# uzh-rpg/dagr

Measured on AMD Instinct MI355X. Metric: events_per_sec, higher is better.
Workload: dtype f32; 1 GPU; dagr-s + --use_image --img_net resnet50, 640x480 synthetic S-uniform, B=8 windows/step x 100000 events (50 ms each), r=7, K=16, events->graph->GNN(+image fusion)->decoded head outputs->confidence mask + NMS (device); image_branch=in-line, engines=3

## Files before the change

### dagr_amd/_lib.py

```python
import ctypes
import os

_HERE = os.path.dirname(os.path.abspath(__file__))
LIB_PATH = os.path.join(_HERE, "lib", "libdagr_hip.so")

c_void_p = ctypes.c_void_p
c_i32 = ctypes.c_int32
c_i64 = ctypes.c_int64
c_size_t = ctypes.c_size_t
c_float = ctypes.c_float


class PoolDesc(ctypes.Structure):
    _fields_ = [("batch_size", c_i32), ("channels", c_i32), ("gx", c_i32), ("gy", c_i32), ("vx", c_float),
                ("vy", c_float), ("inv_w", c_float), ("inv_h", c_float), ("two_max", c_float), ("r00", c_float),
                ("r02", c_float), ("r11", c_float), ("r12", c_float), ("rx", c_i32), ("ry", c_i32), ("aggr", c_i32),
                ("append_pos", c_i32), ("keep_order", c_i32)]


class GraphDesc(ctypes.Structure):
    _fields_ = [("width", c_i32), ("height", c_i32), ("batch_size", c_i32), ("max_neighbors", c_i32),
                ("queue_size", c_i32), ("radius", c_i32), ("delta_t_us", c_i32), ("time_window", c_i32),
                ("max_events", c_i64)]

# ... 111 lines not shown
    "dagr_pool_argmax": (ctypes.c_int, [c_void_p, c_i32, c_void_p, c_i32, c_i32, c_void_p, c_i32, c_i32, c_void_p, c_void_p]),
    "dagr_pool_grad": (ctypes.c_int, [c_void_p, c_i32, c_i32, c_i32, c_void_p, c_void_p, c_void_p, c_i32, c_void_p, c_i32,
                                      c_void_p]),
    "dagr_to_dense_grad": (ctypes.c_int, [c_i32, c_i32, c_void_p, c_void_p, c_float, c_float, c_i32, c_i32, c_i32, c_void_p,
                                          c_void_p, c_i32, c_void_p]),
    "dagr_sample_features": (ctypes.c_int, [c_void_p, c_i32, c_void_p, c_void_p, c_i32, c_void_p, c_i32, c_i32, c_i32,
                                            c_i32, c_i32, c_i32, c_void_p, c_i32, c_i32, c_void_p]),
    "dagr_nms_batched": (ctypes.c_int, [c_void_p, c_void_p, c_void_p, c_void_p, c_i32, c_i32, c_float, c_float, c_void_p,
                                        c_void_p, c_void_p, c_void_p]),
    "dagr_heads_finish": (ctypes.c_int, [ctypes.POINTER(HeadScale), ctypes.POINTER(HeadScale), c_i32, c_i32, c_void_p,
                                         c_void_p, c_void_p]),
    "dagr_heads_finish_detect": (ctypes.c_int, [ctypes.POINTER(HeadScale), ctypes.POINTER(HeadScale), c_i32, c_i32, c_void_p,
                                                c_void_p, c_float, c_float, c_float, c_void_p, c_void_p, c_void_p]),
    "dagr_decode_heads": (ctypes.c_int, [c_void_p, c_i32, c_i32, c_float, c_void_p, c_i32, c_i32, c_float, c_i32, c_i32,
                                         c_void_p, c_void_p]),
    "dagr_postprocess": (ctypes.c_int, [c_void_p, c_i32, c_i32, c_i32, c_float, c_float, c_float, c_void_p, c_void_p,
                                        c_void_p]),
    "dagr_masked_lin": (ctypes.c_int, [c_void_p, c_void_p, c_void_p, c_void_p, c_void_p, c_i32, c_i64, c_i32, c_i32, c_void_p]),
    "dagr_masked_lin_no_bias": (ctypes.c_int, [c_void_p, c_void_p, c_void_p, c_void_p, c_i32, c_i64, c_i32, c_i32, c_void_p]),
    "dagr_masked_isdiff": (ctypes.c_int, [c_void_p, c_void_p, c_void_p, c_float, c_float, c_i64, c_i32, c_void_p]),
    "dagr_masked_inplace_BN": (ctypes.c_int, [c_void_p, c_void_p, c_void_p, c_void_p, c_void_p, c_void_p, c_void_p, c_float,
                                              c_i64, c_i32, c_void_p]),
    "dagr_downsample_events": (ctypes.c_int, [c_void_p, c_void_p, c_void_p, c_i32, c_void_p, c_i32, c_i32, c_void_p,
                                              c_void_p, c_void_p]),
    "dagr_spline_conv_l0_tiles_rows": (ctypes.c_int, [c_i32, c_i32, c_i32, c_i32, c_i32, c_i32, c_i32, c_i32, c_i32, c_float,
                                                      c_float, c_i64, c_i64, c_i32, c_void_p, c_void_p, c_void_p, c_void_p,
                                                      c_i32, c_void_p, c_i32, c_void_p, c_void_p, c_i32, c_void_p, c_i32,
                                                      c_void_p, c_void_p]),
    "dagr_async_graph_append": (ctypes.c_int, [ctypes.POINTER(GraphDesc), c_void_p, c_i64, c_i64, c_void_p, c_void_p,
                                               c_void_p, c_i64, c_void_p, c_i32, c_void_p, c_i32, c_i64, c_void_p, c_void_p,
                                               c_void_p, c_void_p, c_void_p, c_void_p, c_void_p, c_void_p, c_void_p, c_i32,
                                               c_i32, c_i32, c_void_p]),
    "dagr_async_update": (ctypes.c_int, [ctypes.POINTER(AsyncUpdateArgs), c_void_p]),
    "dagr_pool_l0_stream": (ctypes.c_int, [ctypes.POINTER(PoolDesc), c_void_p, c_i32, ctypes.POINTER(GraphDesc), c_void_p,
                                           c_void_p, c_void_p, c_void_p, c_i32, c_void_p, c_void_p, c_i64, c_i64, c_i64,
                                           c_void_p, c_void_p, c_void_p, c_void_p, c_i32, c_i32, c_void_p, c_void_p,
                                           c_void_p, c_void_p, c_void_p, c_void_p, c_void_p, c_i32, c_void_p]),
    "dagr_spline_conv_fused_lds_bytes": (c_size_t, [c_i32, c_i32]),
    "dagr_spline_conv_fused_passes": (c_i32, [c_i32, c_i32]),
    "dagr_spline_conv_fused": (ctypes.c_int, [c_void_p, c_i32, c_void_p, c_void_p, c_void_p, c_void_p, c_i32, c_i32,
                                              c_void_p, c_i32, c_i32, c_i32, c_i32, c_float, c_float, c_void_p,
                                              c_void_p, c_void_p, c_i32, c_i32, c_i32, c_void_p]),
    "dagr_spline_conv_fused_pool": (ctypes.c_int, [c_void_p, c_i32, c_void_p, c_void_p, c_void_p, c_void_p, c_i32, c_i32,
                                                   c_void_p, c_i32, c_i32, c_i32, c_i32, c_float, c_float, c_void_p,
                                                   c_void_p, c_void_p, c_i32, c_i32, c_i32, ctypes.POINTER(PoolDesc),
                                                   c_void_p, c_void_p, c_void_p, c_void_p, c_void_p]),
    "dagr_spline_conv_fused_multi": (ctypes.c_int, [c_void_p, c_i32, c_void_p]),
    "dagr_spline_conv_fused_pair": (ctypes.c_int, [c_void_p, c_i32, c_void_p, c_void_p, c_void_p, c_i32, c_i32, c_i32, c_i32,
                                                   c_float, c_float, c_i32, c_i32, c_void_p, c_void_p, c_void_p, c_void_p,
                                                   c_i32, c_void_p, c_void_p, c_void_p, c_void_p, c_i32, c_void_p]),
    "dagr_gemm_epilogue_workspace_bytes": (c_size_t, []),
    "dagr_gemm_epilogue": (ctypes.c_int, [c_void_p, c_i64, c_i32, c_i64, c_void_p, c_i32, c_void_p, c_void_p, c_i64, c_i32,
                                          c_void_p, c_i64, c_void_p, c_size_t, c_void_p]),
    "dagr_add_relu": (ctypes.c_int, [c_void_p, c_void_p, c_i64, c_void_p]),
    "dagr_bias_relu": (ctypes.c_int, [c_void_p, c_void_p, c_i64, c_i32, c_void_p]),
    "dagr_bias_silu": (ctypes.c_int, [c_void_p, c_void_p, c_i64, c_i32, c_void_p]),
    "dagr_bn_relu_maxpool": (ctypes.c_int, [c_void_p, c_i32, c_i32, c_i32, c_i32, c_void_p, c_void_p, c_void_p, c_void_p]),
    "dagr_gemm_bias_act": (ctypes.c_int, [c_void_p, c_i32, c_void_p, c_i32, c_void_p, c_i32, c_void_p, c_void_p,
                                          c_i32, c_i32, c_i32, c_i32, c_void_p]),
    "dagr_async_flops": (ctypes.c_int, [c_void_p, c_i32, c_void_p, c_void_p, c_void_p, c_void_p, c_void_p, c_i32, c_void_p,
                                        c_void_p]),
    "dagr_viz_workspace_bytes": (c_size_t, [c_i32, c_i32, c_i32]),
    "dagr_viz_render": (ctypes.c_int, [c_void_p, c_i32, c_i32, c_i32, c_void_p, c_i32, c_void_p, c_void_p, c_void_p,
                                       c_void_p, c_i32, c_void_p, c_void_p, c_void_p, c_i32, c_i32, c_void_p, c_i32,
                                       c_void_p, c_void_p, c_void_p, c_size_t, c_void_p]),
}

_lib = None


def lib():
    global _lib
    if _lib is None:
        if not os.path.exists(LIB_PATH):
            raise RuntimeError(
                f"dagr_amd: {LIB_PATH} not found -- build it with `make` (or __graft_entry__.build()). "
                "There is no CPU fallback for the event-graph hot path.")
        handle = ctypes.CDLL(LIB_PATH)
        for name, (res, args) in SIGNATURES.items():
            fn = getattr(handle, name)
            fn.restype = res
            fn.argtypes = args
        _lib = handle
    return _lib


def check(rc, what=""):
    if rc != 0:
        msg = lib().dagr_last_error().decode("utf-8", "replace")
        raise RuntimeError(f"libdagr_hip {what} failed (status {rc}): {msg}")


def ptr(t):
    return None if t is None else c_void_p(t.data_ptr())


def cur_stream(device=None):
    import torch
    return c_void_p(torch.cuda.current_stream(device).cuda_stream)
```

### dagr_amd/csrc/common.hpp

```cpp
#pragma once
#include <hip/hip_runtime.h>
#include <stdint.h>
#include <stdio.h>
#include <stdlib.h>
#include <string>

#include "dagr_hip.h"

namespace dagr {

void set_error(const std::string &msg);

#define DAGR_CHECK_ARG(cond, msg)                                             \
    do {                                                                      \
        if (!(cond)) {                                                        \
            ::dagr::set_error(std::string(__func__) + ": " + (msg));          \
            return DAGR_ERR_INVALID_ARG;                                      \
        }                                                                     \
    } while (0)

#define DAGR_CHECK_HIP(expr)                                                  \
    do {                                                                      \
        hipError_t _e = (expr);                                               \
        if (_e != hipSuccess) {                                               \
// ... 66 lines not shown
        int n = __shfl_up(v, d, 64);
        if (lane >= d) v += n;
    }
    return v;
}

__device__ __forceinline__ int block_exclusive_scan(int v, int *smem, int &total) {
    const int lane = threadIdx.x & 63;
    const int wid = threadIdx.x >> 6;
    int incl = wave_inclusive_scan(v);
    if (lane == 63) smem[wid] = incl;
    __syncthreads();
    int w0 = smem[0], w1 = smem[1], w2 = smem[2], w3 = smem[3];
    __syncthreads();
    int base = (wid > 0 ? w0 : 0) + (wid > 1 ? w1 : 0) + (wid > 2 ? w2 : 0);
    total = w0 + w1 + w2 + w3;
    return base + incl - v;
}

struct XcdSplit {
    int first, end, stride;
};
__device__ __forceinline__ XcdSplit xcd_split(int n_items, int items_per_block, int item_in_block) {
    const int G = gridDim.x;
    const int nx = (G % 8 == 0) ? 8 : 1;
    const int xcd = blockIdx.x % nx, lb = blockIdx.x / nx, bpx = G / nx;
    const int chunk = (n_items + nx - 1) / nx;
    const int begin = xcd * chunk;
    XcdSplit s;
    s.end = min(n_items, begin + chunk);
    s.first = begin + lb * items_per_block + item_in_block;
    s.stride = bpx * items_per_block;
    return s;
}
__device__ __forceinline__ int xcd_block(int n_blocks) {
    const int bpx = (n_blocks + 7) >> 3;
    const int lb = (int)(blockIdx.x >> 3) + (int)(blockIdx.x & 7) * bpx;
    return ((int)(blockIdx.x >> 3) < bpx && lb < n_blocks) ? lb : -1;
}
inline unsigned xcd_grid(int64_t n_blocks) { return (unsigned)((n_blocks + 7) / 8 * 8); }
inline unsigned round_grid8(int64_t g) { return (unsigned)(g <= 8 ? (g < 1 ? 1 : g) : (g + 7) / 8 * 8); }

constexpr int kScanTile = 2048;
size_t scan_scratch_elems(int64_t n);
hipError_t exclusive_scan_i32(int32_t *in, int32_t *out, int64_t n, int32_t *scratch, bool zero_input,
                              hipStream_t stream);
size_t scan_chained_state_bytes(int64_t n);
hipError_t exclusive_scan_i32_chained(int32_t *in, int32_t *out, int64_t n, void *state, bool zero_input,
                                      hipStream_t stream);


hipError_t launch_gemm_mfma(const int32_t *m_ptr, int m_max, const float *A, int lda, const float *Wm, int ldw,
                            const float *bias, float *C, int ldc, int K, int N, int relu, hipStream_t stream);
const int32_t *graph_ws_node_count(const dagr_graph_desc *desc, void *workspace);
struct PixelIndex {
    const int32_t *start;
    const int2 *slot_it;
    const int32_t *slot_xyb;
    const int32_t *n_nodes;
    const int32_t *unsorted;
    int W, H;
    __host__ __device__ int segment(int x, int yb) const { return x + W * yb; }
    __host__ __device__ int row_begin(int yb) const { return W * yb; }
};
void graph_ws_index(const dagr_graph_desc *desc, void *workspace, PixelIndex *out);

}
```

### dagr_amd/csrc/gemm_lt.hip

```cpp
#include <hipblaslt/hipblaslt.h>

#include <map>
#include <tuple>

#include "common.hpp"

namespace dagr {
namespace {

struct LtPlan {
    hipblasLtMatmulDesc_t desc = nullptr;
    hipblasLtMatrixLayout_t a = nullptr, b = nullptr, c = nullptr, d = nullptr;
    hipblasLtMatmulAlgo_t algo;
    size_t workspace = 0;
};

hipblasLtHandle_t lt_handle() {
    static hipblasLtHandle_t h = [] {
        hipblasLtHandle_t hh = nullptr;
        if (hipblasLtCreate(&hh) != HIPBLAS_STATUS_SUCCESS) hh = nullptr;
        return hh;
    }();
    return h;
}

}
}

using namespace dagr;

extern "C" size_t dagr_gemm_epilogue_workspace_bytes(void) { return (size_t)64 << 20; }

extern "C" int dagr_gemm_epilogue(const float *A, int64_t M, int32_t K, int64_t lda, const float *Wt, int32_t N,
                                  const float *bias, const float *R, int64_t ldr, int32_t act, float *D, int64_t ldd,
                                  void *workspace, size_t workspace_bytes, void *stream) {
    DAGR_CHECK_ARG(M >= 0 && K >= 1 && N >= 1 && lda >= K && ldd >= N && (!R || ldr >= N) && (act == 0 || act == 1), "bad sizes");
    if (M == 0) return DAGR_OK;
    DAGR_CHECK_ARG(A && Wt && D, "NULL pointer");
    hipblasLtHandle_t h = lt_handle();
    if (!h) { set_error("dagr_gemm_epilogue: hipblasLtCreate failed"); return DAGR_ERR_HIP; }
    using Key = std::tuple<int64_t, int, int, int64_t, int64_t, int64_t, int, int, int>;
    static thread_local std::map<Key, LtPlan> plans;
    const Key key{M, K, N, lda, R ? ldr : -1, ldd, act, bias ? 1 : 0, R ? 1 : 0};
    auto it = plans.find(key);
    if (it == plans.end()) {
        LtPlan p;
#define LT_OK(expr)                                                                                        \
    do {                                                                                                   \
        if ((expr) != HIPBLAS_STATUS_SUCCESS) { set_error("dagr_gemm_epilogue: " #expr " failed"); return DAGR_ERR_HIP; } \
    } while (0)
        LT_OK(hipblasLtMatmulDescCreate(&p.desc, HIPBLAS_COMPUTE_32F, HIP_R_32F));
        const hipblasOperation_t op_n = HIPBLAS_OP_N;
        LT_OK(hipblasLtMatmulDescSetAttribute(p.desc, HIPBLASLT_MATMUL_DESC_TRANSA, &op_n, sizeof(op_n)));
        LT_OK(hipblasLtMatmulDescSetAttribute(p.desc, HIPBLASLT_MATMUL_DESC_TRANSB, &op_n, sizeof(op_n)));
        hipblasLtEpilogue_t epi = act ? (bias ? HIPBLASLT_EPILOGUE_RELU_BIAS : HIPBLASLT_EPILOGUE_RELU)
                                      : (bias ? HIPBLASLT_EPILOGUE_BIAS : HIPBLASLT_EPILOGUE_DEFAULT);
        LT_OK(hipblasLtMatmulDescSetAttribute(p.desc, HIPBLASLT_MATMUL_DESC_EPILOGUE, &epi, sizeof(epi)));
        if (bias) {
            const hipDataType bt = HIP_R_32F;
            LT_OK(hipblasLtMatmulDescSetAttribute(p.desc, HIPBLASLT_MATMUL_DESC_BIAS_DATA_TYPE, &bt, sizeof(bt)));
            LT_OK(hipblasLtMatmulDescSetAttribute(p.desc, HIPBLASLT_MATMUL_DESC_BIAS_POINTER, &bias, sizeof(bias)));
        }
        LT_OK(hipblasLtMatrixLayoutCreate(&p.a, HIP_R_32F, (uint64_t)N, (uint64_t)K, (int64_t)N));
        LT_OK(hipblasLtMatrixLayoutCreate(&p.b, HIP_R_32F, (uint64_t)K, (uint64_t)M, lda));
        LT_OK(hipblasLtMatrixLayoutCreate(&p.c, HIP_R_32F, (uint64_t)N, (uint64_t)M, R ? ldr : ldd));
        LT_OK(hipblasLtMatrixLayoutCreate(&p.d, HIP_R_32F, (uint64_t)N, (uint64_t)M, ldd));
        hipblasLtMatmulPreference_t pref = nullptr;
        LT_OK(hipblasLtMatmulPreferenceCreate(&pref));
        const uint64_t max_ws = workspace ? (uint64_t)workspace_bytes : 0;
        LT_OK(hipblasLtMatmulPreferenceSetAttribute(pref, HIPBLASLT_MATMUL_PREF_MAX_WORKSPACE_BYTES, &max_ws, sizeof(max_ws)));
        constexpr int kCand = 16;
        hipblasLtMatmulHeuristicResult_t res[kCand];
        int found = 0;
        const hipblasStatus_t st = hipblasLtMatmulAlgoGetHeuristic(h, p.desc, p.a, p.b, p.c, p.d, pref, kCand, res, &found);
        hipblasLtMatmulPreferenceDestroy(pref);
        if (st != HIPBLAS_STATUS_SUCCESS || found < 1) {
            set_error("dagr_gemm_epilogue: the library offers no kernel for this GEMM + epilogue");
            return DAGR_ERR_UNSUPPORTED;
        }
        int best = 0;
        hipStreamCaptureStatus cap = hipStreamCaptureStatusNone;
        (void)hipStreamIsCapturing((hipStream_t)stream, &cap);
        if (found > 1 && cap == hipStreamCaptureStatusNone) {
            hipEvent_t e0, e1;
            if (hipEventCreate(&e0) == hipSuccess && hipEventCreate(&e1) == hipSuccess) {
                const float alpha = 1.0f, beta = R ? 1.0f : 0.0f;
                float best_ms = 0.f;
                for (int c = 0; c < found; c++) {
                    if (res[c].workspaceSize > workspace_bytes) continue;
                    bool ok = true;
                    float ms = 0.f;
                    for (int rep = 0; rep < 3 && ok; rep++) {
                        if (rep == 1) (void)hipEventRecord(e0, (hipStream_t)stream);
                        ok = hipblasLtMatmul(h, p.desc, &alpha, Wt, p.a, A, p.b, &beta, R ? (const void *)R : (const void *)D,
                                             p.c, D, p.d, &res[c].algo, workspace, workspace_bytes,
                                             (hipStream_t)stream) == HIPBLAS_STATUS_SUCCESS;
                    }
                    (void)hipEventRecord(e1, (hipStream_t)stream);
                    if (hipEventSynchronize(e1) != hipSuccess || !ok) continue;
                    (void)hipEventElapsedTime(&ms, e0, e1);
                    if (best_ms == 0.f || ms < best_ms) { best_ms = ms; best = c; }
                }
                (void)hipEventDestroy(e0);
                (void)hipEventDestroy(e1);
            }
        }
        p.algo = res[best].algo;
        p.workspace = res[best].workspaceSize;
        it = plans.emplace(key, p).first;
#undef LT_OK
    }
    LtPlan &p = it->second;
    if (bias && hipblasLtMatmulDescSetAttribute(p.desc, HIPBLASLT_MATMUL_DESC_BIAS_POINTER, &bias, sizeof(bias)) !=
                    HIPBLAS_STATUS_SUCCESS) {
        set_error("dagr_gemm_epilogue: setting the bias pointer failed");
        return DAGR_ERR_HIP;
    }
    DAGR_CHECK_ARG(p.workspace <= workspace_bytes, "workspace too small for the selected kernel");
    const float alpha = 1.0f, beta = R ? 1.0f : 0.0f;
    const hipblasStatus_t st = hipblasLtMatmul(h, p.desc, &alpha, Wt, p.a, A, p.b, &beta, R ? (const void *)R : (const void *)D,
                                               p.c, D, p.d, &p.algo, workspace, workspace_bytes, (hipStream_t)stream);
    if (st != HIPBLAS_STATUS_SUCCESS) {
        set_error("dagr_gemm_epilogue: hipblasLtMatmul failed");
        return DAGR_ERR_HIP;
    }
    return DAGR_OK;
}
```

### dagr_amd/engine.py

```python
import contextlib
import ctypes
import gc
import types

import numpy as np
import torch

from . import _lib
from .graph.ev_graph import WindowGraphBuilder

FUSED_PASSES_MAX_NODES = 1600


def _f32(v):
    return float(torch.as_tensor(v, dtype=torch.float32))


def _same_domain(a, b):
    return (a["rx"], a["ry"], a["den_x"], a["den_y"]) == (b["rx"], b["ry"], b["den_x"], b["den_y"]) \
        and torch.equal(a["remap"], b["remap"])


def _bn_affine(bn):
    m = bn.module
# ... 31 lines not shown
def _pack_generic(convs, norms, skip=None, relu=True, device="cuda"):
    cols, biases = [], []
    cin = convs[0].in_channels
    for conv, norm in zip(convs, norms):
        W = conv.weight.detach().float()
        root = conv.lin.weight.detach().float()
        cout = W.shape[2]
        if norm is not None:
            scale, shift = _bn_affine(norm)
        else:
            scale, shift = torch.ones(cout, device=W.device), torch.zeros(cout, device=W.device)
        if conv.bias is not None:
            shift = shift + conv.bias.detach().float() * scale
        block = torch.cat([W.reshape(25 * cin, cout), root.t()], 0) * scale.view(1, -1)
        if skip is not None:
            lin, norm_skip = skip
            s_scale, s_shift = _bn_affine(norm_skip)
            block = torch.cat([block, lin.mlp.weight.detach().float().t() * s_scale.view(1, -1)], 0)
            shift = shift + s_shift
        cols.append(block)
        biases.append(shift)
    cskip = skip[0].mlp.in_features if skip is not None else 0
    return _ConvPack(cin, cskip, torch.cat(cols, 1).to(device), torch.cat(biases).to(device), relu)


def _pack_l0(conv, norm, win, skip=None, device="cuda", cols_in=None, cols_skip=None):
    win_x, tx, win_y, ty = win
    W = conv.weight.detach().float()
    cin, cout = W.shape[1], W.shape[2]
    if cout != 16:
        raise NotImplementedError("the level-0 kernels are specialised for 16 output channels (base_width = 0.5)")
    cols_in = list(range(cin)) if cols_in is None else list(cols_in)
    scale, shift = _bn_affine(norm)
    rows = []
    for b in range(ty):
        for a in range(tx):
            rows.append(W[(win_x + a) + 5 * (win_y + b)][cols_in] * scale.view(1, -1))
    rows.append(conv.lin.weight.detach().float().t()[cols_in] * scale.view(1, -1))
    cskip = 0
    if skip is not None:
        lin, norm_skip = skip
        s_scale, s_shift = _bn_affine(norm_skip)
        ws = lin.mlp.weight.detach().float().t()
        if cols_skip is not None:
            ws = ws[list(cols_skip)]
        rows.append(ws * s_scale.view(1, -1))
        shift = shift + s_shift
        cskip = lin.mlp.in_features
    return cin, cskip, torch.cat(rows, 0).contiguous().to(device), shift.contiguous().to(device)


class _Conv1x1Gemm(torch.nn.Module):

    def __init__(self, conv, relu=False):
        super().__init__()
        cout, cin = conv.weight.shape[:2]
        self.stride = conv.stride[0]
        self.relu = relu
        self.register_buffer("wt", conv.weight.detach().reshape(cout, cin).t().contiguous())
        self.register_buffer("b", conv.bias.detach().clone() if conv.bias is not None else torch.zeros(cout, device=conv.weight.device))

    def forward(self, x, residual=None):
        if self.stride != 1:
            x = x[:, :, ::self.stride, ::self.stride]
        B, C, H, W = x.shape
        a = x.permute(0, 2, 3, 1).reshape(-1, C)
        N = self.wt.shape[1]
        r = None if residual is None else residual.permute(0, 2, 3, 1)
        if _LT["ok"] and a.is_cuda and a.dtype == torch.float32 and a.stride(1) == 1 \
                and (r is None or (r.is_contiguous() and tuple(r.shape) == (B, H, W, N))):
            y = torch.empty((a.shape[0], N), dtype=torch.float32, device=a.device)
            ws = _lt_workspace(a.device)
            act = 1 if (self.relu or r is not None) else 0
            rc = _lib.lib().dagr_gemm_epilogue(_lib.ptr(a), a.shape[0], C, a.stride(0), _lib.ptr(self.wt), N,
                                               _lib.ptr(self.b), _lib.ptr(r), N, act, _lib.ptr(y), N, _lib.ptr(ws),
                                               ws.numel(), _lib.cur_stream(a.device))
            if rc == 0:
                return y.view(B, H, W, -1).permute(0, 3, 1, 2)
            _LT["ok"] = False
        if residual is not None:
            y = torch.addmm(self.b, a, self.wt).view(B, H, W, -1).permute(0, 3, 1, 2)
            return _add_relu_(y, residual)
        y = torch._addmm_activation(self.b, a, self.wt) if self.relu else torch.addmm(self.b, a, self.wt)
        return y.view(B, H, W, -1).permute(0, 3, 1, 2)


_LT = {"ok": True, "ws": {}}


def _lt_workspace(device):
    key = str(device)
    if key not in _LT["ws"]:
        _LT["ws"][key] = torch.empty(int(_lib.lib().dagr_gemm_epilogue_workspace_bytes()), dtype=torch.uint8, device=device)
    return _LT["ws"][key]


def _gemmify_1x1(module):
    for name, child in list(module.named_children()):
        if isinstance(child, torch.nn.Conv2d) and child.kernel_size == (1, 1) and child.groups == 1 \
                and child.padding == (0, 0) and child.stride[0] == child.stride[1]:
            setattr(module, name, _Conv1x1Gemm(child))
        else:
            _gemmify_1x1(child)


def _add_relu_(y, z):
    if y.is_cuda and y.dtype == torch.float32 and z.dtype == torch.float32 and y.shape == z.shape \
            and y.stride() == z.stride() and y.data_ptr() % 16 == 0 and z.data_ptr() % 16 == 0 \
            and (y.is_contiguous() or y.is_contiguous(memory_format=torch.channels_last)):
        _lib.check(_lib.lib().dagr_add_relu(_lib.ptr(y), _lib.ptr(z), y.numel(), _lib.cur_stream(y.device)), "add_relu")
        return y
    return torch.relu_(y.add_(z))


def _bias_relu_(y, bias):
    C = y.shape[1]
    if y.is_cuda and y.dtype == torch.float32 and C % 4 == 0 and y.is_contiguous(memory_format=torch.channels_last) \
            and y.data_ptr() % 16 == 0 and bias.data_ptr() % 16 == 0:
        _lib.check(_lib.lib().dagr_bias_relu(_lib.ptr(y), _lib.ptr(bias), y.numel(), C, _lib.cur_stream(y.device)),
                   "bias_relu")
        return y
    return torch.relu_(y.add_(bias.view(1, -1, 1, 1)))


def _baseconv_forward(m, x):
    y = m.conv(x)
    b = m._bias
    C = y.shape[1]
    if y.is_cuda and y.dtype == torch.float32 and C % 4 == 0 and y.is_contiguous(memory_format=torch.channels_last) \
            and y.data_ptr() % 16 == 0 and b.data_ptr() % 16 == 0:
        _lib.check(_lib.lib().dagr_bias_silu(_lib.ptr(y), _lib.ptr(b), y.numel(), C, _lib.cur_stream(y.device)),
                   "bias_silu")
        return y
    return torch.nn.functional.silu(y.add_(b.view(1, -1, 1, 1)), inplace=True)


def _conv_bias_relu(blk, name, x):
    conv = getattr(blk, name)
    b = getattr(blk, "_" + name + "_bias", None)
    out = conv(x)
    if b is not None:
        return _bias_relu_(out, b)
    if getattr(conv, "relu", False):
        return out
    return blk.relu(out)


def _bottleneck_forward(blk, x):
    identity = x if blk.downsample is None else blk.downsample(x)
    out = _conv_bias_relu(blk, "conv1", x)
    out = _conv_bias_relu(blk, "conv2", out)
    if isinstance(blk.conv3, _Conv1x1Gemm):
        return blk.conv3(out, residual=identity)
    return _add_relu_(blk.conv3(out), identity)


def _resnet_features_forward(net, x, emit=None):
    emit = emit or (lambda name, t: None)
    c1 = net.conv1(x)
    emit("conv1", c1)
    mp = net.maxpool
    ok = (c1.is_cuda and c1.dtype == torch.float32 and c1.is_contiguous(memory_format=torch.channels_last)
          and c1.shape[1] % 4 == 0 and mp.kernel_size == 3 and mp.stride == 2 and mp.padding == 1
          and mp.dilation == 1 and not mp.ceil_mode)
    if ok:
        B, C, H, W = c1.shape
        scale, shift = net._stem_affine
        y = torch.empty((B, C, (H - 1) // 2 + 1, (W - 1) // 2 + 1), dtype=c1.dtype, device=c1.device,
                        memory_format=torch.channels_last)
        _lib.check(_lib.lib().dagr_bn_relu_maxpool(_lib.ptr(c1), B, H, W, C, _lib.ptr(scale), _lib.ptr(shift), _lib.ptr(y),
                                                   _lib.cur_stream(c1.device)), "bn_relu_maxpool")
    else:
        y = net.maxpool(net.relu(net.bn1(c1)))
    l1 = net.layer1(y)
    emit("layer1", l1)
    l2 = net.layer2(l1)
    emit("layer2", l2)
    l3 = net.layer3(l2)
    emit("layer3", l3)
    l4 = net.layer4(l3)
    emit("layer4", l4)
    return dict(conv1=c1, layer1=l1, layer2=l2, layer3=l3, layer4=l4)


def _basicblock_forward(blk, x):
    identity = x if blk.downsample is None else blk.downsample(x)
    out = _conv_bias_relu(blk, "conv1", x)
    return _add_relu_(blk.conv2(out), identity)


class _Level:

    def __init__(self, T, cin, cout, device, cf_next=0):
        self.T = T
        self.e_cap = T * 64
        i32 = dict(dtype=torch.int32, device=device)
        f32 = dict(dtype=torch.float32, device=device)
        self.x = torch.zeros((T, (cin + 3) // 4 * 4), **f32)
# ... 422 lines not shown
        if self._feat_ready is not None:
            ready = self._feat_ready.get(id(fmap))
            if ready is None:
                raise RuntimeError("pipelined window: a sampled feature map has no ready-event (the image branch did not "
                                   "announce it) -- reading it would race with the image stream")
            torch.cuda.current_stream(self.device).wait_event(ready)
        Bf, C, h, w = fmap.shape
        nhwc = fmap.permute(0, 2, 3, 1)
        if not nhwc.is_contiguous():
            nhwc = nhwc.contiguous()
        self._keep.append(nhwc)
        _lib.check(self.L.dagr_sample_features(n_ptr, n_max, _lib.ptr(pos), _lib.ptr(batch), b64, _lib.ptr(nhwc), Bf, h,
                                               w, C, self.W, self.H, _lib.ptr(out), out.shape[1], coff,
                                               _lib.cur_stream(self.device)), "sample_features")

    def _fold_image_branch(self):
        import copy
        from torch.nn.utils.fusion import fuse_conv_bn_eval
        bb, head = self.model.backbone, self.model.head
        net = copy.deepcopy(bb.net).eval()
        cnn = copy.deepcopy(head.cnn_head).eval()

        def fold_block(blk):
            for ci, bi in (("conv1", "bn1"), ("conv2", "bn2"), ("conv3", "bn3")):
                if hasattr(blk, ci):
                    setattr(blk, ci, fuse_conv_bn_eval(getattr(blk, ci), getattr(blk, bi)))
                    setattr(blk, bi, torch.nn.Identity())
            if blk.downsample is not None:
                blk.downsample = torch.nn.Sequential(fuse_conv_bn_eval(blk.downsample[0], blk.downsample[1]))
        for name in ("layer1", "layer2", "layer3", "layer4"):
            for blk in getattr(net.module, name):
                fold_block(blk)
        for m in cnn.modules():
            if hasattr(m, "conv") and hasattr(m, "bn") and isinstance(m.bn, torch.nn.BatchNorm2d):
                m.conv = fuse_conv_bn_eval(m.conv, m.bn)
                m.bn = torch.nn.Identity()
                if isinstance(getattr(m, "act", None), torch.nn.SiLU) and m.conv.bias is not None:
                    m._bias = m.conv.bias.detach().clone().contiguous()
                    m.conv.bias = None
                    m.forward = types.MethodType(_baseconv_forward, m)
        net = net.to(memory_format=torch.channels_last)
        cnn = cnn.to(memory_format=torch.channels_last)
        for blkname in ("layer1", "layer2", "layer3", "layer4"):
            _gemmify_1x1(getattr(net.module, blkname))
            for blk in getattr(net.module, blkname):
                relu_convs = ("conv1", "conv2") if hasattr(blk, "conv3") else ("conv1",)
                for cname in relu_convs:
                    conv = getattr(blk, cname)
                    if isinstance(conv, _Conv1x1Gemm):
                        conv.relu = True
                    elif isinstance(conv, torch.nn.Conv2d) and conv.bias is not None:
                        setattr(blk, "_" + cname + "_bias", conv.bias.detach().clone().contiguous())
                        conv.bias = None
                blk.forward = types.MethodType(_bottleneck_forward if hasattr(blk, "conv3") else _basicblock_forward,
                                               blk)
        bn = net.module.bn1
        scale = (bn.weight.detach().float() / torch.sqrt(bn.running_var.detach().float() + bn.eps)).contiguous()
        shift = (bn.bias.detach().float() - bn.running_mean.detach().float() * scale).contiguous()
        net.module._stem_affine = (scale, shift)
        net.module.forward_features = types.MethodType(_resnet_features_forward, net.module)
        _gemmify_1x1(net.feature_dconv)
        _gemmify_1x1(net.output_dconv)
        self._net_f, self._cnn_f = net, cnn

    def _image_branch(self, image, on_feature=None):
        if self._net_f is None:
            self._fold_image_branch()
        bb, head = types.SimpleNamespace(net=self._net_f), types.SimpleNamespace(cnn_head=self._cnn_f)
        x = image.contiguous(memory_format=torch.channels_last)
        net = self._net_f
        if on_feature is not None:
            feats = [None] * len(net.feature_layers)

            def emit(name, t):
                if name in net.feature_layers:
                    j = net.feature_layers.index(name)
                    feats[j] = net.feature_dconv[j](t) if len(net.feature_dconv) > 0 else t
                    on_feature(j, feats[j])
            d = _resnet_features_forward(net.module, x, emit)
            outs = [d[l] for l in net.output_layers]
            if len(net.output_dconv) > 0:
                outs = [dconv(o) for o, dconv in zip(outs, net.output_dconv)]
        else:
            feats, outs = bb.net(x)
        outs = outs[-self.num_scales:]
        resized = [torch.nn.functional.interpolate(f, o) for f, o in zip(outs, self.out_sizes)]
        return feats, head.cnn_head(resized)

    def stage_image(self, image):
        self._keep = []
        self._img_feats, self._cnn_out = self._image_branch(image)

    def image_async(self, image, stream=None):
        cur = torch.cuda.current_stream(self.device)
        if stream is not None:
            self._img_stream = stream
        if self._img_stream is None:
            self._img_stream = torch.cuda.Stream(self.device)
        s = self._img_stream
        s.wait_stream(cur)
        with torch.cuda.stream(s):
            feats, cnn_out = self._image_branch(image)
            ev = torch.cuda.Event()
            ev.record(s)
        return feats, cnn_out, ev

    def _consume_image_handle(self, handle):
        feats, cnn_out, ev = handle
        cur = torch.cuda.current_stream(self.device)
        cur.wait_event(ev)
        for t in list(feats) + [o for v in cnn_out.values() for o in v]:
            t.record_stream(cur)
        self._keep = []
        self._img_feats, self._cnn_out = feats, cnn_out

# ... 536 lines not shown
```

### include/dagr_hip.h

```cpp
#ifndef DAGR_HIP_H
#define DAGR_HIP_H

#include <stddef.h>
#include <stdint.h>

#ifdef __cplusplus
extern "C" {
#endif

typedef enum {
    DAGR_OK = 0,
    DAGR_ERR_INVALID_ARG = -1,
    DAGR_ERR_HIP = -2,
    DAGR_ERR_WORKSPACE = -3,
    DAGR_ERR_UNSUPPORTED = -4
} dagr_status;

const char *dagr_last_error(void);
int dagr_version(void);
int dagr_device_count(void);

int dagr_format_events(const int16_t *xy , const int32_t *t , const int8_t *p ,
                       int64_t N, int32_t width, int32_t height, int32_t time_window,
                       float *pos_out , float *feat_out , void *stream);
// ... 221 lines not shown

int dagr_add_relu(float *y, const float *z, int64_t n, void *stream);
int dagr_bias_relu(float *y_nhwc, const float *bias, int64_t n, int32_t C, void *stream);
int dagr_bias_silu(float *y_nhwc, const float *bias, int64_t n, int32_t C, void *stream);
int dagr_bn_relu_maxpool(const float *x_nhwc, int32_t B, int32_t H, int32_t W, int32_t C, const float *scale,
                         const float *shift, float *y_nhwc, void *stream);

int dagr_sample_features(const int32_t *n_ptr, int32_t n_max, const float *pos, const void *batch,
                         int32_t batch_is_int64, const float *feat_nhwc, int32_t B, int32_t h, int32_t w, int32_t C,
                         int32_t width, int32_t height, float *out, int32_t ldo, int32_t coff, void *stream);

int dagr_nms_batched(const float *boxes, const float *scores, const int32_t *cls, const uint8_t *valid,
                     int32_t B, int32_t A, float iou_threshold, float class_offset,
                     int32_t *order_out, int32_t *keep_out, int32_t *n_keep, void *stream);

typedef struct dagr_head_scale {
    const int32_t *n_ptr; int32_t n_max;
    const float *pred; int32_t ld;
    const float *pos; const int32_t *batch;
    float vx, vy, stride; int32_t Hc, Wc;
    const float *cnn[3]; int32_t cnn_stride[3][4];
    float *dense;
} dagr_head_scale;
int dagr_heads_finish(const dagr_head_scale *scale0, const dagr_head_scale *scale1, int32_t batch_size, int32_t channels,
                      float *out, int32_t *status, void *stream);
int dagr_heads_finish_detect(const dagr_head_scale *scale0, const dagr_head_scale *scale1, int32_t batch_size,
                             int32_t channels, float *out, int32_t *status, float conf_threshold, float iou_threshold,
                             float class_offset, float *det, int32_t *n_keep, void *stream);
int dagr_decode_heads(const float *dense0, int32_t H0, int32_t W0, float stride0, const float *dense1, int32_t H1,
                      int32_t W1, float stride1, int32_t B, int32_t channels, float *out, void *stream);

int dagr_postprocess(const float *pred, int32_t B, int32_t A, int32_t num_classes, float conf_threshold,
                     float iou_threshold, float class_offset, float *det, int32_t *n_keep, void *stream);

int dagr_masked_lin(const int64_t *indices, const float *x_in, float *x_out, const float *weight, const float *bias,
                    int32_t add, int64_t K, int32_t Cin, int32_t Cout, void *stream);
int dagr_masked_lin_no_bias(const int64_t *indices, const float *x_in, float *x_out, const float *weight, int32_t add,
                            int64_t K, int32_t Cin, int32_t Cout, void *stream);
int dagr_masked_isdiff(int64_t *indices, const float *x_old, const float *x_new, float atol, float rtol, int64_t K,
                       int32_t C, void *stream);
int dagr_masked_inplace_BN(const int64_t *indices, const float *x, float *x_out, const float *running_mean,
                           const float *running_var, const float *weight, const float *bias, float eps, int64_t K,
                           int32_t C, void *stream);

int dagr_downsample_events(const int32_t *order, const int32_t *run_cell, const int32_t *run_end, int32_t n_runs,
                           const int8_t *polarity, int32_t fx, int32_t fy, float *change_map, uint8_t *keep,
                           void *stream);

size_t dagr_gemm_epilogue_workspace_bytes(void);
int dagr_gemm_epilogue(const float *A, int64_t M, int32_t K, int64_t lda, const float *Wt, int32_t N, const float *bias,
                       const float *R, int64_t ldr, int32_t act, float *D, int64_t ldd, void *workspace,
                       size_t workspace_bytes, void *stream);

enum { DAGR_FLOPS_ZERO = 0, DAGR_FLOPS_CONV = 1, DAGR_FLOPS_LINEAR = 2, DAGR_FLOPS_POOL = 3, DAGR_FLOPS_CARTESIAN = 4 };
typedef struct dagr_flops_module {
    int32_t kind, level, cin, cout, root, bias;
} dagr_flops_module;
int dagr_async_flops(const int32_t *deg, int32_t n_events, const int32_t *counts1, const int32_t *counts2,
                     const int32_t *counts3, const int32_t *counts4, const dagr_flops_module *mods, int32_t n_mods,
                     int64_t *out, void *stream);

size_t dagr_viz_workspace_bytes(int32_t F, int32_t H, int32_t W);
int dagr_viz_render(const uint8_t *images, int32_t n_images, int32_t H, int32_t W, const int32_t *frame_image, int32_t F,
                    const int32_t *ev_x, const int32_t *ev_y, const int8_t *ev_p, const int32_t *ev_ptr, int32_t n_events,
                    const double *alpha, const int32_t *boxes, const int32_t *box_ptr, int32_t n_boxes, int32_t linewidth,
                    const uint8_t *colors, int32_t n_colors, uint8_t *out, int32_t *status, void *workspace,
                    size_t workspace_bytes, void *stream);

int dagr_spiral_offsets(int32_t n, int32_t *dx_host, int32_t *dy_host);

#ifdef __cplusplus
}
#endif
#endif
```

Before: 148.2 million events/s.

## Add custom MFMA implicit-GEMM conv kernel with autotuned variants for ResNet image branch

Adds a custom HIP kernel using fp32 MFMA 32x32x2 for 3x3 implicit-GEMM convolutions and 1x1 GEMMs. It offers tile sizes and split-K options, with a reduction kernel that applies bias, residual and ReLU. The ResNet image branch times each variant against the existing cuDNN/MIOpen conv and hipBLASLt GEMM on first use and keeps the fastest. It also shares one workspace buffer across modules. This targets conv and GEMM overhead in the image branch, at the cost of one-time autotuning and a new code path that must handle padding and alignment correctly.

```diff
diff --git a/dagr_amd/_lib.py b/dagr_amd/_lib.py
--- a/dagr_amd/_lib.py
+++ b/dagr_amd/_lib.py
@@ -187,6 +187,9 @@
     "dagr_gemm_epilogue_workspace_bytes": (c_size_t, []),
     "dagr_gemm_epilogue": (ctypes.c_int, [c_void_p, c_i64, c_i32, c_i64, c_void_p, c_i32, c_void_p, c_void_p, c_i64, c_i32,
                                           c_void_p, c_i64, c_void_p, c_size_t, c_void_p]),
+    "dagr_img_conv_variants": (ctypes.c_int, [c_i64, c_i32, c_i32, c_i32, c_void_p, c_void_p]),
+    "dagr_img_conv": (ctypes.c_int, [c_void_p, c_i32, c_i32, c_i32, c_i32, c_i64, c_i32, c_i32, c_void_p, c_i32, c_void_p,
+                                     c_void_p, c_i64, c_i32, c_void_p, c_i64, c_i32, c_void_p, c_size_t, c_void_p]),
     "dagr_add_relu": (ctypes.c_int, [c_void_p, c_void_p, c_i64, c_void_p]),
     "dagr_bias_relu": (ctypes.c_int, [c_void_p, c_void_p, c_i64, c_i32, c_void_p]),
     "dagr_bias_silu": (ctypes.c_int, [c_void_p, c_void_p, c_i64, c_i32, c_void_p]),
@@ -200,6 +203,8 @@
                                        c_void_p, c_i32, c_void_p, c_void_p, c_void_p, c_i32, c_i32, c_void_p, c_i32,
                                        c_void_p, c_void_p, c_void_p, c_size_t, c_void_p]),
 }
+
+IMG_CONV_MAX_VARIANTS = 12
 
 _lib = None
 
diff --git a/dagr_amd/csrc/common.hpp b/dagr_amd/csrc/common.hpp
--- a/dagr_amd/csrc/common.hpp
+++ b/dagr_amd/csrc/common.hpp
@@ -142,6 +142,10 @@
 
 hipError_t launch_gemm_mfma(const int32_t *m_ptr, int m_max, const float *A, int lda, const float *Wm, int ldw,
                             const float *bias, float *C, int ldc, int K, int N, int relu, hipStream_t stream);
+size_t img_conv_workspace_bytes(int64_t M, int Cin, int N, int taps, int variant);
+int launch_img_conv(const float *A, int64_t B, int H, int W, int Cin, int64_t lda, int taps, int stride, const float *Wp,
+                    int N, const float *bias, const float *R, int64_t ldr, int act, float *D, int64_t ldd, int variant,
+                    void *workspace, size_t workspace_bytes, hipStream_t stream);
 const int32_t *graph_ws_node_count(const dagr_graph_desc *desc, void *workspace);
 struct PixelIndex {
     const int32_t *start;
diff --git a/dagr_amd/csrc/gemm_lt.hip b/dagr_amd/csrc/gemm_lt.hip
--- a/dagr_amd/csrc/gemm_lt.hip
+++ b/dagr_amd/csrc/gemm_lt.hip
@@ -13,6 +13,7 @@
     hipblasLtMatrixLayout_t a = nullptr, b = nullptr, c = nullptr, d = nullptr;
     hipblasLtMatmulAlgo_t algo;
     size_t workspace = 0;
+    int own_variant = -1;
 };
 
 hipblasLtHandle_t lt_handle() {
@@ -81,7 +82,17 @@
         int best = 0;
         hipStreamCaptureStatus cap = hipStreamCaptureStatusNone;
         (void)hipStreamIsCapturing((hipStream_t)stream, &cap);
-        if (found > 1 && cap == hipStreamCaptureStatusNone) {
+        bool own_ok[DAGR_IMG_CONV_MAX_VARIANTS];
+        int own_found = 0;
+        for (int v = 0; v < DAGR_IMG_CONV_MAX_VARIANTS; v++) {
+            const size_t need = M < ((int64_t)1 << 31) ? img_conv_workspace_bytes(M, K, N, 1, v) : (size_t)-1;
+            own_ok[v] = need != (size_t)-1 && need <= (workspace ? workspace_bytes : 0) && lda % 4 == 0 && ldd % 4 == 0 &&
+                        (!R || ldr % 4 == 0) && ((uintptr_t)A % 16 == 0) && ((uintptr_t)Wt % 16 == 0) &&
+                        ((uintptr_t)D % 16 == 0) && ((uintptr_t)bias % 16 == 0) && ((uintptr_t)R % 16 == 0) &&
+                        ((uintptr_t)workspace % 16 == 0);
+            own_found += own_ok[v];
+        }
+        if (found + own_found > 1 && cap == hipStreamCaptureStatusNone) {
             hipEvent_t e0, e1;
             if (hipEventCreate(&e0) == hipSuccess && hipEventCreate(&e1) == hipSuccess) {
                 const float alpha = 1.0f, beta = R ? 1.0f : 0.0f;
@@ -101,6 +112,20 @@
                     (void)hipEventElapsedTime(&ms, e0, e1);
                     if (best_ms == 0.f || ms < best_ms) { best_ms = ms; best = c; }
                 }
+                for (int v = 0; v < DAGR_IMG_CONV_MAX_VARIANTS; v++) {
+                    if (!own_ok[v]) continue;
+                    bool ok = true;
+                    float ms = 0.f;
+                    for (int rep = 0; rep < 3 && ok; rep++) {
+                        if (rep == 1) (void)hipEventRecord(e0, (hipStream_t)stream);
+                        ok = launch_img_conv(A, M, 1, 1, K, lda, 1, 1, Wt, N, bias, R, ldr, act, D, ldd, v, workspace,
+                                             workspace_bytes, (hipStream_t)stream) == DAGR_OK;
+                    }
+                    (void)hipEventRecord(e1, (hipStream_t)stream);
+                    if (hipEventSynchronize(e1) != hipSuccess || !ok) continue;
+                    (void)hipEventElapsedTime(&ms, e0, e1);
+                    if (best_ms == 0.f || ms < best_ms) { best_ms = ms; p.own_variant = v; }
+                }
                 (void)hipEventDestroy(e0);
                 (void)hipEventDestroy(e1);
             }
@@ -111,6 +136,9 @@
 #undef LT_OK
     }
     LtPlan &p = it->second;
+    if (p.own_variant >= 0)
+        return launch_img_conv(A, M, 1, 1, K, lda, 1, 1, Wt, N, bias, R, ldr, act, D, ldd, p.own_variant, workspace,
+                               workspace_bytes, (hipStream_t)stream);
     if (bias && hipblasLtMatmulDescSetAttribute(p.desc, HIPBLASLT_MATMUL_DESC_BIAS_POINTER, &bias, sizeof(bias)) !=
                     HIPBLAS_STATUS_SUCCESS) {
         set_error("dagr_gemm_epilogue: setting the bias pointer failed");
diff --git a/dagr_amd/csrc/img_gemm.hip b/dagr_amd/csrc/img_gemm.hip
--- /dev/null
+++ b/dagr_amd/csrc/img_gemm.hip
@@ -0,0 +1,316 @@
+#include "common.hpp"
+
+namespace dagr {
+namespace {
+
+typedef float f32x16 __attribute__((ext_vector_type(16)));
+typedef float f32x4 __attribute__((ext_vector_type(4)));
+
+constexpr int kBK = 32;
+constexpr int kLdA = kBK + 1;
+
+struct ImgTile { int bm, bn; };
+constexpr ImgTile kTiles[3] = {{128, 128}, {128, 64}, {64, 64}};
+constexpr int kSplits[4] = {1, 2, 4, 8};
+constexpr int kVariants = 12;
+static_assert(kVariants == DAGR_IMG_CONV_MAX_VARIANTS, "header and kernel table disagree");
+
+struct ImgArgs {
+    const float *A, *Wp, *bias, *R;
+    float *D, *part;
+    int64_t M, lda, ldr, ldd;
+    int Cin, N, act;
+    int H, W, Ho, Wo, stride;
+    int tiles_m, tiles_n, splits, chunks;
+};
+
+constexpr size_t img_lds_bytes(int bm, int bn) { return (size_t)2 * (bm * kLdA + kBK * bn) * sizeof(float); }
+
+template <int BM, int BN, bool CONV>
+__global__ __launch_bounds__(256) void k_img_gemm(const ImgArgs p) {
+    constexpr int WM = BM / 2, WN = BN / 2;
+    constexpr int MI = WM / 32, NI = WN / 32;
+    constexpr int AV = BM / 32, BV = BN / 32;
+    constexpr int BQ = BN / 4;
+    constexpr int BROWS = 256 / BQ;
+    constexpr int A_FLOATS = BM * kLdA, STAGE = A_FLOATS + kBK * BN;
+    extern __shared__ __attribute__((aligned(16))) float lds[];
+
+    const int n_blocks = p.tiles_m * p.tiles_n * p.splits;
+    const int lb = xcd_block(n_blocks);
+    if (lb < 0) return;
+    const int tn = lb % p.tiles_n, tm = (lb / p.tiles_n) % p.tiles_m, z = lb / (p.tiles_n * p.tiles_m);
+    const int t = threadIdx.x, lane = t & 63, wid = t >> 6;
+    const int wm = wid >> 1, wn = wid & 1;
+
+    const int a_kq = t & 7, a_r0 = t >> 3;
+    int64_t a_base[AV];
+    uint32_t a_mask[AV];
+#pragma unroll
+    for (int i = 0; i < AV; i++) {
+        const int64_t m = (int64_t)tm * BM + a_r0 + 32 * i;
+        a_base[i] = 0;
+        a_mask[i] = 0;
+        if (m < p.M) {
+            if (CONV) {
+                const int hw = p.Ho * p.Wo;
+                const int b = (int)(m / hw), rem = (int)(m - (int64_t)b * hw);
+                const int y = rem / p.Wo, x = rem - y * p.Wo;
+                const int iy0 = y * p.stride - 1, ix0 = x * p.stride - 1;
+                a_base[i] = (((int64_t)b * p.H + iy0) * p.W + ix0) * p.lda;
+                uint32_t mk = 0;
+#pragma unroll
+                for (int dy = 0; dy < 3; dy++)
+#pragma unroll
+                    for (int dx = 0; dx < 3; dx++)
+                        if (iy0 + dy >= 0 && iy0 + dy < p.H && ix0 + dx >= 0 && ix0 + dx < p.W) mk |= 1u << (dy * 3 + dx);
+                a_mask[i] = mk;
+            } else {
+                a_base[i] = m * p.lda;
+                a_mask[i] = 1u;
+            }
+        }
+    }
+    const int b_nq = t % BQ, b_k0 = t / BQ;
+    const float *w_col = p.Wp + (int64_t)tn * BN + b_nq * 4;
+
+    const int cpt = p.Cin / kBK;
+    const int c_begin = (int)((int64_t)p.chunks * z / p.splits), c_end = (int)((int64_t)p.chunks * (z + 1) / p.splits);
+
+    uint32_t a_ok = 0;
+    f32x4 ra[AV], rb[BV];
+#define IMG_LOAD_STEP(c_)                                                                                         \
+    {                                                                                                             \
+        const int tap_ = CONV ? (c_) / cpt : 0;                                                                   \
+        const int kc_ = ((c_) - tap_ * cpt) * kBK;                                                                \
+        int64_t shift_ = kc_ + a_kq * 4;                                                                          \
+        if (CONV) shift_ += ((int64_t)(tap_ / 3) * p.W + (tap_ % 3)) * p.lda;                                     \
+        _Pragma("unroll") for (int i = 0; i < AV; i++) {                                                          \
+            const bool ok_ = (a_mask[i] >> tap_) & 1u;                                                            \
+            const f32x4 v_ = *reinterpret_cast<const f32x4 *>(p.A + (ok_ ? a_base[i] + shift_ : (int64_t)0));   \
+            ra[i] = v_;                                                                                           \
+            a_ok = ok_ ? (a_ok | (1u << i)) : (a_ok & ~(1u << i));                                                \
+        }                                                                                                         \
+        const float *wrow_ = w_col + ((int64_t)tap_ * p.Cin + kc_ + b_k0) * p.N;                                  \
+        _Pragma("unroll") for (int i = 0; i < BV; i++)                                                            \
+            rb[i] = *reinterpret_cast<const f32x4 *>(wrow_ + (int64_t)(BROWS * i) * p.N);                        \
+    }
+#define IMG_STORE_STEP(stage_)                                                                                    \
+    {                                                                                                             \
+        _Pragma("unroll") for (int i = 0; i < AV; i++) {                                                          \
+            float *d_ = (stage_) + (a_r0 + 32 * i) * kLdA + a_kq * 4;                                             \
+            const bool ok_ = (a_ok >> i) & 1u;        \
+            d_[0] = ok_ ? ra[i].x : 0.f; d_[1] = ok_ ? ra[i].y : 0.f;                                             \
+            d_[2] = ok_ ? ra[i].z : 0.f; d_[3] = ok_ ? ra[i].w : 0.f;                                             \
+        }                                                                                                         \
+        _Pragma("unroll") for (int i = 0; i < BV; i++)                                                            \
+            *reinterpret_cast<f32x4 *>((stage_) + A_FLOATS + (b_k0 + BROWS * i) * BN + b_nq * 4) = rb[i];        \
+    }
+
+    f32x16 acc[MI][NI];
+#pragma unroll
+    for (int mi = 0; mi < MI; mi++)
+#pragma unroll
+        for (int ni = 0; ni < NI; ni++)
+#pragma unroll
+            for (int r = 0; r < 16; r++) acc[mi][ni][r] = 0.f;
+
+    const int fr = lane & 31, fh = lane >> 5;
+    int cur = 0;
+    IMG_LOAD_STEP(c_begin)
+    IMG_STORE_STEP(lds)
+    __syncthreads();
+    for (int c = c_begin; c < c_end; c++) {
+        const int cn = c + 1 < c_end ? c + 1 : c;
+        IMG_LOAD_STEP(cn)
+        __builtin_amdgcn_sched_barrier(0);
+        const float *as = lds + cur * STAGE + (wm * WM + fr) * kLdA + fh;
+        const float *bs = lds + cur * STAGE + A_FLOATS + fh * BN + wn * WN + fr;
+        float a[2][MI], b[2][NI];
+#pragma unroll
+        for (int mi = 0; mi < MI; mi++) a[0][mi] = as[mi * 32 * kLdA];
+#pragma unroll
+        for (int ni = 0; ni < NI; ni++) b[0][ni] = bs[ni * 32];
+#pragma unroll
+        for (int kk = 0; kk < kBK; kk += 2) {
+            const int q = (kk >> 1) & 1;
+            if (kk + 2 < kBK) {
+#pragma unroll
+                for (int mi = 0; mi < MI; mi++) a[q ^ 1][mi] = as[mi * 32 * kLdA + kk + 2];
+#pragma unroll
+                for (int ni = 0; ni < NI; ni++) b[q ^ 1][ni] = bs[(kk + 2) * BN + ni * 32];
+            }
+#pragma unroll
+            for (int mi = 0; mi < MI; mi++)
+#pragma unroll
+                for (int ni = 0; ni < NI; ni++)
+                    acc[mi][ni] = __builtin_amdgcn_mfma_f32_32x32x2f32(a[q][mi], b[q][ni], acc[mi][ni], 0, 0, 0);
+        }
+        __builtin_amdgcn_sched_barrier(0);
+        IMG_STORE_STEP(lds + (cur ^ 1) * STAGE)
+        __syncthreads();
+        cur ^= 1;
+    }
+#undef IMG_LOAD_STEP
+#undef IMG_STORE_STEP
+
+#pragma unroll
+    for (int mi = 0; mi < MI; mi++) {
+#pragma unroll
+        for (int r = 0; r < 16; r++) {
+            const int64_t row = (int64_t)tm * BM + wm * WM + mi * 32 + (r & 3) + 8 * (r >> 2) + 4 * fh;
+            if (row >= p.M) continue;
+#pragma unroll
+            for (int ni = 0; ni < NI; ni++) {
+                const int col = tn * BN + wn * WN + ni * 32 + fr;
+                float v = acc[mi][ni][r];
+                if (p.splits > 1) {
+                    p.part[((int64_t)z * p.M + row) * p.N + col] = v;
+                } else {
+                    if (p.bias) v += p.bias[col];
+                    if (p.R) v += p.R[row * p.ldr + col];
+                    if (p.act) v = fmaxf(v, 0.f);
+                    p.D[row * p.ldd + col] = v;
+                }
+            }
+        }
+    }
+}
+
+__global__ __launch_bounds__(256) void k_img_reduce(const ImgArgs p) {
+    const int nq = p.N / 4;
+    const int64_t total = p.M * nq;
+    const int64_t slab = p.M * (int64_t)p.N;
+    for (int64_t i = (int64_t)blockIdx.x * blockDim.x + threadIdx.x; i < total; i += (int64_t)gridDim.x * blockDim.x) {
+        const int64_t row = i / nq;
+        const int col = (int)(i - row * nq) * 4;
+        const float *src = p.part + row * p.N + col;
+        float4 s = *reinterpret_cast<const float4 *>(src);
+        for (int z = 1; z < p.splits; z++) {
+            const float4 q = *reinterpret_cast<const float4 *>(src + z * slab);
+            s.x += q.x; s.y += q.y; s.z += q.z; s.w += q.w;
+        }
+        if (p.bias) {
+            const float4 q = *reinterpret_cast<const float4 *>(p.bias + col);
+            s.x += q.x; s.y += q.y; s.z += q.z; s.w += q.w;
+        }
+        if (p.R) {
+            const float4 q = *reinterpret_cast<const float4 *>(p.R + row * p.ldr + col);
+            s.x += q.x; s.y += q.y; s.z += q.z; s.w += q.w;
+        }
+        if (p.act) { s.x = fmaxf(s.x, 0.f); s.y = fmaxf(s.y, 0.f); s.z = fmaxf(s.z, 0.f); s.w = fmaxf(s.w, 0.f); }
+        *reinterpret_cast<float4 *>(p.D + row * p.ldd + col) = s;
+    }
+}
+
+template <int BM, int BN, bool CONV>
+hipError_t launch_tile(const ImgArgs &p, hipStream_t stream) {
+    constexpr size_t lds = img_lds_bytes(BM, BN);
+    static thread_local bool lds_set = false;
+    if (!lds_set) {
+        const hipError_t e = hipFuncSetAttribute((const void *)k_img_gemm<BM, BN, CONV>,
+                                                 hipFuncAttributeMaxDynamicSharedMemorySize, (int)lds);
+        if (e != hipSuccess) return e;
+        lds_set = true;
+    }
+    const unsigned grid = xcd_grid((int64_t)p.tiles_m * p.tiles_n * p.splits);
+    hipLaunchKernelGGL((k_img_gemm<BM, BN, CONV>), dim3(grid), dim3(256), lds, stream, p);
+    return hipGetLastError();
+}
+
+bool aligned16(const void *q) { return ((uintptr_t)q & 15) == 0; }
+
+}
+
+size_t img_conv_workspace_bytes(int64_t M, int Cin, int N, int taps, int variant) {
+    if (variant < 0 || variant >= kVariants || M < 1 || Cin < 64 || Cin > 2048 || N < 64 || N > 2048 || Cin % 64 || N % 64 ||
+        (taps != 1 && taps != 9))
+        return (size_t)-1;
+    const ImgTile tile = kTiles[variant / 4];
+    const int S = kSplits[variant % 4];
+    if (N % tile.bn != 0 || S > taps * Cin / kBK) return (size_t)-1;
+    if (ceil_div(M, tile.bm) * (N / tile.bn) * S > (int64_t)1 << 24) return (size_t)-1;
+    return S > 1 ? (size_t)S * (size_t)M * (size_t)N * sizeof(float) : 0;
+}
+
+int launch_img_conv(const float *A, int64_t B, int H, int W, int Cin, int64_t lda, int taps, int stride, const float *Wp,
+                    int N, const float *bias, const float *R, int64_t ldr, int act, float *D, int64_t ldd, int variant,
+                    void *workspace, size_t workspace_bytes, hipStream_t stream) {
+    const bool conv = taps == 9;
+    const int Ho = conv ? (H - 1) / stride + 1 : H, Wo = conv ? (W - 1) / stride + 1 : W;
+    const int64_t M = B * Ho * Wo;
+    const size_t need = img_conv_workspace_bytes(M, Cin, N, taps, variant);
+    if (need == (size_t)-1) {
+        set_error("dagr_img_conv: no such variant for this shape (Cin, Cout multiples of 64 in 64..2048, Cout a multiple of the tile)");
+        return DAGR_ERR_UNSUPPORTED;
+    }
+    if (lda % 4 || !aligned16(A) || !aligned16(Wp) ||
+        (need > 0 && (ldd % 4 || !aligned16(D) || (bias && !aligned16(bias)) || (R && (ldr % 4 || !aligned16(R)))))) {
+        set_error("dagr_img_conv: operands must be 16-byte aligned with row strides that are multiples of 4");
+        return DAGR_ERR_UNSUPPORTED;
+    }
+    if (need > 0 && (!workspace || workspace_bytes < need || !aligned16(workspace))) {
+        set_error("dagr_img_conv: workspace too small for this split variant");
+        return DAGR_ERR_WORKSPACE;
+    }
+    const ImgTile tile = kTiles[variant / 4];
+    ImgArgs p{};
+    p.A = A; p.Wp = Wp; p.bias = bias; p.R = R; p.D = D; p.part = (float *)workspace;
+    p.M = M; p.lda = lda; p.ldr = ldr; p.ldd = ldd;
+    p.Cin = Cin; p.N = N; p.act = act;
+    p.H = H; p.W = W; p.Ho = Ho; p.Wo = Wo; p.stride = stride;
+    p.tiles_m = (int)ceil_div(M, tile.bm); p.tiles_n = N / tile.bn;
+    p.splits = kSplits[variant % 4]; p.chunks = taps * Cin / kBK;
+    hipError_t e = hipSuccess;
+    switch (variant / 4) {
+        case 0: e = conv ? launch_tile<128, 128, true>(p, stream) : launch_tile<128, 128, false>(p, stream); break;
+        case 1: e = conv ? launch_tile<128, 64, true>(p, stream) : launch_tile<128, 64, false>(p, stream); break;
+        default: e = conv ? launch_tile<64, 64, true>(p, stream) : launch_tile<64, 64, false>(p, stream); break;
+    }
+    if (e == hipSuccess && p.splits > 1) {
+        const int64_t quads = M * (N / 4);
+        const unsigned grid = (unsigned)(ceil_div(quads, 256) < 4096 ? ceil_div(quads, 256) : 4096);
+        hipLaunchKernelGGL(k_img_reduce, dim3(grid), dim3(256), 0, stream, p);
+        e = hipGetLastError();
+    }
+    if (e != hipSuccess) {
+        set_error(std::string("dagr_img_conv: launch -> ") + hipGetErrorString(e));
+        return DAGR_ERR_HIP;
+    }
+    return DAGR_OK;
+}
+
+}
+
+using namespace dagr;
+
+extern "C" int dagr_img_conv_variants(int64_t M, int32_t Cin, int32_t Cout, int32_t taps, int32_t *n_variants,
+                                      size_t *workspace_bytes) {
+    DAGR_CHECK_ARG(n_variants && workspace_bytes, "NULL pointer");
+    DAGR_CHECK_ARG(M >= 1 && (taps == 1 || taps == 9), "bad sizes");
+    int usable = 0;
+    for (int v = 0; v < kVariants; v++) {
+        workspace_bytes[v] = img_conv_workspace_bytes(M, Cin, Cout, taps, v);
+        usable += workspace_bytes[v] != (size_t)-1;
+    }
+    *n_variants = kVariants;
+    if (!usable) {
+        set_error("dagr_img_conv_variants: Cin and Cout must be multiples of 64 in 64..2048");
+        return DAGR_ERR_UNSUPPORTED;
+    }
+    return DAGR_OK;
+}
+
+extern "C" int dagr_img_conv(const float *A, int32_t B, int32_t H, int32_t W, int32_t Cin, int64_t lda, int32_t taps,
+                             int32_t stride, const float *Wp, int32_t Cout, const float *bias, const float *R, int64_t ldr,
+                             int32_t act, float *D, int64_t ldd, int32_t variant, void *workspace, size_t workspace_bytes,
+                             void *stream) {
+    DAGR_CHECK_ARG(B >= 0 && H >= 0 && W >= 0 && Cin >= 1 && Cout >= 1 && lda >= Cin && ldd >= Cout && (!R || ldr >= Cout) &&
+                       (act == 0 || act == 1) && (taps == 1 || taps == 9) && (stride == 1 || (taps == 9 && stride == 2)),
+                   "bad sizes");
+    if ((int64_t)B * H * W == 0) return DAGR_OK;
+    DAGR_CHECK_ARG((int64_t)B * H * W < ((int64_t)1 << 31), "map too large");
+    DAGR_CHECK_ARG(A && Wp && D, "NULL pointer");
+    return launch_img_conv(A, B, H, W, Cin, lda, taps, stride, Wp, Cout, bias, R, ldr, act, D, ldd, variant, workspace,
+                           workspace_bytes, (hipStream_t)stream);
+}
diff --git a/dagr_amd/engine.py b/dagr_amd/engine.py
--- a/dagr_amd/engine.py
+++ b/dagr_amd/engine.py
@@ -107,6 +107,8 @@
 
 class _Conv1x1Gemm(torch.nn.Module):
 
+    _ws = None
+
     def __init__(self, conv, relu=False):
         super().__init__()
         cout, cin = conv.weight.shape[:2]
@@ -125,7 +127,7 @@
         if _LT["ok"] and a.is_cuda and a.dtype == torch.float32 and a.stride(1) == 1 \
                 and (r is None or (r.is_contiguous() and tuple(r.shape) == (B, H, W, N))):
             y = torch.empty((a.shape[0], N), dtype=torch.float32, device=a.device)
-            ws = _lt_workspace(a.device)
+            ws = self._ws if self._ws is not None else _lt_workspace(a.device)
             act = 1 if (self.relu or r is not None) else 0
             rc = _lib.lib().dagr_gemm_epilogue(_lib.ptr(a), a.shape[0], C, a.stride(0), _lib.ptr(self.wt), N,
                                                _lib.ptr(self.b), _lib.ptr(r), N, act, _lib.ptr(y), N, _lib.ptr(ws),
@@ -193,12 +195,62 @@
 def _conv_bias_relu(blk, name, x):
     conv = getattr(blk, name)
     b = getattr(blk, "_" + name + "_bias", None)
+    wp = getattr(blk, "_" + name + "_wp", None)
+    if wp is not None and b is not None:
+        out = _conv3x3_own(conv, wp, b, x, blk._img_ws)
+        if out is not None:
+            return out
     out = conv(x)
     if b is not None:
         return _bias_relu_(out, b)
     if getattr(conv, "relu", False):
         return out
     return blk.relu(out)
+
+
+_IMG3 = {"sel": {}, "used": {}}
+
+
+def _conv3x3_own(conv, wp, bias, x, ws):
+    B, Cin, H, W = x.shape
+    Cout, s = wp.shape[1], conv.stride[0]
+    if not (x.is_cuda and x.dtype == torch.float32 and x.is_contiguous(memory_format=torch.channels_last)
+            and x.data_ptr() % 16 == 0):
+        return None
+    key = (B, H, W, Cin, Cout, s)
+    L = _lib.lib()
+    Ho, Wo = (H - 1) // s + 1, (W - 1) // s + 1
+
+    def own(v):
+        y = torch.empty((B, Cout, Ho, Wo), dtype=torch.float32, device=x.device, memory_format=torch.channels_last)
+        _lib.check(L.dagr_img_conv(_lib.ptr(x), B, H, W, Cin, Cin, 9, s, _lib.ptr(wp), Cout, _lib.ptr(bias), None, 0, 1,
+                                   _lib.ptr(y), Cout, v, _lib.ptr(ws), ws.numel(), _lib.cur_stream(x.device)), "img_conv")
+        return y
+
+    choice = _IMG3["sel"].get(key)
+    if choice is None:
+        if torch.cuda.is_current_stream_capturing():
+            return None
+        need = (ctypes.c_size_t * _lib.IMG_CONV_MAX_VARIANTS)()
+        n = ctypes.c_int32(0)
+        cands = [-1]
+        if L.dagr_img_conv_variants(B * Ho * Wo, Cin, Cout, 9, ctypes.byref(n), need) == 0:
+            cands += [v for v in range(n.value) if need[v] <= ws.numel()]
+        e0, e1 = torch.cuda.Event(enable_timing=True), torch.cuda.Event(enable_timing=True)
+        best = None
+        for v in cands:
+            for rep in range(3):
+                if rep == 1:
+                    e0.record()
+                _bias_relu_(conv(x), bias) if v < 0 else own(v)
+            e1.record()
+            e1.synchronize()
+            ms = e0.elapsed_time(e1)
+            if best is None or ms < best:
+                best, choice = ms, v
+        _IMG3["sel"][key] = choice
+    _IMG3["used"][key] = choice
+    return None if choice < 0 else own(choice)
 
 
 def _bottleneck_forward(blk, x):
@@ -727,6 +779,11 @@
                     elif isinstance(conv, torch.nn.Conv2d) and conv.bias is not None:
                         setattr(blk, "_" + cname + "_bias", conv.bias.detach().clone().contiguous())
                         conv.bias = None
+                        cout, cin = conv.weight.shape[:2]
+                        if conv.kernel_size == (3, 3) and conv.padding == (1, 1) and conv.dilation == (1, 1) \
+                                and conv.groups == 1 and conv.stride in ((1, 1), (2, 2)) and cin % 64 == 0 and cout % 64 == 0:
+                            setattr(blk, "_" + cname + "_wp",
+                                    conv.weight.detach().permute(2, 3, 1, 0).reshape(9 * cin, cout).contiguous())
                 blk.forward = types.MethodType(_bottleneck_forward if hasattr(blk, "conv3") else _basicblock_forward,
                                                blk)
         bn = net.module.bn1
@@ -736,6 +793,12 @@
         net.module.forward_features = types.MethodType(_resnet_features_forward, net.module)
         _gemmify_1x1(net.feature_dconv)
         _gemmify_1x1(net.output_dconv)
+        ws = torch.empty(int(_lib.lib().dagr_gemm_epilogue_workspace_bytes()), dtype=torch.uint8, device=self.device)
+        for m in list(net.modules()) + list(cnn.modules()):
+            if isinstance(m, _Conv1x1Gemm):
+                m._ws = ws
+            elif hasattr(m, "_conv1_wp") or hasattr(m, "_conv2_wp"):
+                m._img_ws = ws
         self._net_f, self._cnn_f = net, cnn
 
     def _image_branch(self, image, on_feature=None):
diff --git a/include/dagr_hip.h b/include/dagr_hip.h
--- a/include/dagr_hip.h
+++ b/include/dagr_hip.h
@@ -297,6 +297,12 @@
                        const float *R, int64_t ldr, int32_t act, float *D, int64_t ldd, void *workspace,
                        size_t workspace_bytes, void *stream);
 
+#define DAGR_IMG_CONV_MAX_VARIANTS 12
+int dagr_img_conv_variants(int64_t M, int32_t Cin, int32_t Cout, int32_t taps, int32_t *n_variants, size_t *workspace_bytes);
+int dagr_img_conv(const float *A, int32_t B, int32_t H, int32_t W, int32_t Cin, int64_t lda, int32_t taps, int32_t stride,
+                  const float *Wp, int32_t Cout, const float *bias, const float *R, int64_t ldr, int32_t act, float *D,
+                  int64_t ldd, int32_t variant, void *workspace, size_t workspace_bytes, void *stream);
+
 enum { DAGR_FLOPS_ZERO = 0, DAGR_FLOPS_CONV = 1, DAGR_FLOPS_LINEAR = 2, DAGR_FLOPS_POOL = 3, DAGR_FLOPS_CARTESIAN = 4 };
 typedef struct dagr_flops_module {
     int32_t kind, level, cin, cout, root, bias;
```

Result: slower. 142.5 million events/s (-3.8%).
